# biscuitzb/COEB-SLAM

Measured on AMD Instinct MI355X. Metric: frames/sec ORB extract+match @640x480/1000 kp; 1/2/4/8 GPU + %HBM roofline, higher is better.
Workload: dtype u8; 1 GPU; 640x480, 8-level pyramid, 1000 kp, extract + Hamming match to prev frame (BASELINE configs[1]); width=640, height=480, nfeatures=1000, nlevels=8, halo_frames_per_rank=1, pipelines_per_gpu=3, streams_per_gpu=1, ranks=single, parallelism=frame-sharded x1 (no collectives), hw_queues=4, side_stream=own, side_stream_created=with the context

## Files before the change

coeb-slam_amd/csrc/coeb_extract.hip:

```cpp
#include <type_traits>
#include <cmath>
#include <hip/hip_runtime.h>

#include "coeb_internal.hpp"

namespace {

constexpr int kThreads = 256;
constexpr int kWaves = kThreads / 64;

__device__ __forceinline__ int lane_id() { return __lane_id(); }
__device__ __forceinline__ int wave_id() { return __builtin_amdgcn_readfirstlane(threadIdx.x >> 6); }
__device__ __forceinline__ void wave_sync_lds()
{
    __builtin_amdgcn_fence(__ATOMIC_RELEASE, "wavefront");
    __builtin_amdgcn_wave_barrier();
    __builtin_amdgcn_fence(__ATOMIC_ACQUIRE, "wavefront");
}
typedef unsigned int u32x4 __attribute__((ext_vector_type(4)));

__device__ __forceinline__ uint64_t lanemask_lt() { return (1ull << lane_id()) - 1ull; }

__device__ __forceinline__ int wave_sum(int v)
{
// ... 345 lines not shown
    uint32_t sel[2], coef[2];
    const int d0 = min((int)cx, dw - 1);
    const uint32_t wb = (uint32_t)(xofs[d0] & ~3);
    const uint32_t wb1 = (uint32_t)min((int)wb + 4, sp - 4);
#pragma unroll
    for (int k = 0; k < 2; k++) {
        const int d = min((int)cx + k, dw - 1);
        const int o = xofs[d] - (int)wb;
        const int a = alpha[d];
        const uint32_t a0 = d >= xmax ? 2048u : (uint32_t)(a & 0xFFFF), a1 = d >= xmax ? 0u : (uint32_t)a >> 16;
        coef[k] = a0 | (a1 << 16);
        sel[k] = (uint32_t)o | 0x0c00u | ((uint32_t)(o + 1) << 16) | 0x0c000000u;
    }
    const __amdgpu_buffer_rsrc_t rs =
        __builtin_amdgcn_make_buffer_rsrc((void*)(src + (int64_t)f * src_fs), 0, 0x7fffffff, 0x00020000);
    const __amdgpu_buffer_rsrc_t rd =
        __builtin_amdgcn_make_buffer_rsrc((void*)(dst + (int64_t)f * dst_fs), 0, 0x7fffffff, 0x00020000);
    const bool edge = ox + PR_COLS > dw - 1, tail = ox + PR_COLS > xs;
    const int* band = bands + (oy / PR_ROWS) * kPyrBandInts;
    const int4 bd = *reinterpret_cast<const int4*>(band);
    if (bd.x != kPyrBandGeneric) {
#define COEB_PYR_PATTERN(P, LAST) pyr_rows_pattern<P, LAST>(rs, rd, wb, wb1, sel, coef, band, bd.y, bd.z, sp, dp, cx, dw, xs)
        if (edge || tail) {
            switch (bd.x) {
            case 0: COEB_PYR_PATTERN(0, true); break;
            case 1: COEB_PYR_PATTERN(1, true); break;
            case 2: COEB_PYR_PATTERN(2, true); break;
            case 3: COEB_PYR_PATTERN(3, true); break;
            default: COEB_PYR_PATTERN(4, true); break;
            }
        } else {
            switch (bd.x) {
            case 0: COEB_PYR_PATTERN(0, false); break;
            case 1: COEB_PYR_PATTERN(1, false); break;
            case 2: COEB_PYR_PATTERN(2, false); break;
            case 3: COEB_PYR_PATTERN(3, false); break;
            default: COEB_PYR_PATTERN(4, false); break;
            }
        }
#undef COEB_PYR_PATTERN
        return;
    }
    uint32_t w[PR_ROWS][4];
#pragma unroll
    for (int r = 0; r < PR_ROWS; r++) {
        const int4 yr = yrow[min(oy + r, dh - 1)];
        w[r][0] = __builtin_amdgcn_raw_buffer_load_b32(rs, wb, yr.x, 0);
        w[r][1] = __builtin_amdgcn_raw_buffer_load_b32(rs, wb1, yr.x, 0);
        w[r][2] = __builtin_amdgcn_raw_buffer_load_b32(rs, wb, yr.y, 0);
        w[r][3] = __builtin_amdgcn_raw_buffer_load_b32(rs, wb1, yr.y, 0);
    }
    if (tail) {
        if (edge) pyr_rows_out<true, true>(w, sel, coef, yrow, rd, oy, dh, cx, dw, xs);
        else pyr_rows_out<true, false>(w, sel, coef, yrow, rd, oy, dh, cx, dw, xs);
    } else {
        if (edge) pyr_rows_out<false, true>(w, sel, coef, yrow, rd, oy, dh, cx, dw, xs);
        else pyr_rows_out<false, false>(w, sel, coef, yrow, rd, oy, dh, cx, dw, xs);
    }
}

constexpr int kBlurCols = 56;

__device__ __forceinline__ int reflect101(int p, int len)
{
    if (len == 1) return 0;
    while (p < 0 || p >= len) p = p < 0 ? -p : 2 * len - p - 2;
    return p;
}

struct BlurWork {
    int L;
    int item0, item1;
    int item_off[COEB_MAXL + 1];
    int nstrips[COEB_MAXL];
    int bh[COEB_MAXL];
    int nquads[COEB_MAXL];
    int brows;
};


template <bool kRemap = true>
__device__ __forceinline__ int2 block_xy()
{
    const int gx = gridDim.x;
    if (!kRemap) return make_int2(blockIdx.x, blockIdx.y);
    const int n = gx * gridDim.y, p = blockIdx.x + gx * blockIdx.y;
    const int q = n >> 3, r = n & 7, x = p & 7, k = p >> 3;
    const int lg = x * q + min(x, r) + k;
    return make_int2(lg % gx, lg / gx);
}

__device__ __forceinline__ uint32_t dpp_shr1(uint32_t v)
{
    return (uint32_t)__builtin_amdgcn_mov_dpp((int)v, 0x111, 0xf, 0xf, false);
}
__device__ __forceinline__ uint32_t dpp_shl1(uint32_t v)
{
    return (uint32_t)__builtin_amdgcn_mov_dpp((int)v, 0x101, 0xf, 0xf, false);
}

__device__ __forceinline__ int reflect_row(int r, int h)
{
    int rr = r < 0 ? -r : r;
    rr = rr >= h ? 2 * h - 2 - rr : rr;
    return rr < 0 ? 0 : rr;
}

constexpr int kBlurQuad = 4 * kBlurCols;
constexpr int kBlurPitch = kBlurQuad + 16;
static_assert(kBlurQuad % 16 == 0, "a wave item must cover whole 16-column tiles");

__global__ __launch_bounds__(kThreads) void k_blur_rows(const Plan* __restrict__ P, ExtractBufs b, BlurWork bw)
{
    __shared__ __attribute__((aligned(16))) uint8_t s_tile[kWaves][8 * kBlurPitch];
    const int2 bxy = block_xy();
    const int f = bxy.y;
    const int item = bw.item0 + bxy.x * kWaves + wave_id();
    if (item >= bw.item1) return;
    int l = 0;
    while (l + 1 < bw.L && item >= bw.item_off[l + 1]) l++;
    const int it = item - bw.item_off[l];
    const int nq = bw.nquads[l];
    const int quad = it % nq, band = it / nq;
    const LevelGeom& g = P->lv[l];
    const int w = g.w, h = g.h, sp = g.pitch, dp = g.bpitch;
    const int lane = lane_id(), grp = lane >> 4, gl = lane & 15;
    const int y0 = band * bw.brows, y1 = min(h, y0 + bw.brows);
    const int x = (quad * 4 + grp) * kBlurCols - 4 + gl * 4;
    const bool produce = gl >= 1 && gl <= 14 && x < w;
    const int xbase = quad * kBlurQuad;
    uint8_t* tl = s_tile[wave_id()];
    int cq[4];
#pragma unroll
    for (int q = 0; q < 4; q++) cq[q] = reflect101(min(x + q, w + 2), w);
    const int a = min(min(min(cq[0], cq[1]), min(cq[2], cq[3])), w - 4);
    const uint32_t sel0 = 0x0c000c00u | (uint32_t)(cq[0] - a) | ((uint32_t)(cq[1] - a) << 16);
    const uint32_t sel1 = 0x0c000c00u | (uint32_t)(cq[2] - a) | ((uint32_t)(cq[3] - a) << 16);
    const __amdgpu_buffer_rsrc_t rs =
        __builtin_amdgcn_make_buffer_rsrc((void*)level_ptr(P, b, f, l), 0, 0x7fffffff, 0x00020000);
    const __amdgpu_buffer_rsrc_t rd =
        __builtin_amdgcn_make_buffer_rsrc((void*)(b.blur + (int64_t)f * P->blur_stride + g.blur_off), 0, 0x7fffffff,
                                          0x00020000);
    const int k0 = P->gauss[0], k1 = P->gauss[1], k2 = P->gauss[2], k3 = P->gauss[3];
    const us2 K0 = pk2(k0, k0), K1 = pk2(k1, k1), K2 = pk2(k2, k2), K3 = pk2(k3, k3);
    const us2 W_l01_0 = pk2(0, k0), W_l23_0 = pk2(k1, k2), W_c01_0 = pk2(k3, k2), W_c23_0 = pk2(k1, k0);
    const us2 W_l23_1 = pk2(k0, k1), W_c01_1 = pk2(k2, k3), W_c23_1 = pk2(k2, k1), W_r01_1 = pk2(k0, 0);
    const us2 W_l23_2 = pk2(0, k0), W_c01_2 = pk2(k1, k2), W_c23_2 = pk2(k3, k2), W_r01_2 = pk2(k1, k0);
    const us2 W_c01_3 = pk2(k0, k1), W_c23_3 = pk2(k2, k3), W_r01_3 = pk2(k2, k1), W_r23_3 = pk2(k0, 0);
    const uint32_t rnd = 1u << 15;
    const int nfull = (y1 - y0) >> 3, tail = (y1 - y0) & 7;
    uint32_t R0[8], R1[8];
    auto take = [&](int s, uint32_t raw) {
        R0[s] = __builtin_amdgcn_perm(0u, raw, sel0);
        R1[s] = __builtin_amdgcn_perm(0u, raw, sel1);
    };
    typedef __attribute__((address_space(3))) uint32_t* lds_u32;
    lds_u32 trow = (lds_u32)(tl + (produce ? x - xbase : kBlurQuad + 8 * (grp & 1) + 4 * (gl & 1)));
    asm volatile("" : "+v"(trow));
    auto out_row = [&](int s, int k) {
        const int s0 = (s + 2) & 7, s1 = (s + 3) & 7, s2 = (s + 4) & 7, s3 = (s + 5) & 7, s4 = (s + 6) & 7,
                  s5 = (s + 7) & 7, s6 = s;
        const us2 v01 = K3 * as_us2(R0[s3]) + K2 * (as_us2(R0[s2]) + as_us2(R0[s4])) +
                        K1 * (as_us2(R0[s1]) + as_us2(R0[s5])) + K0 * (as_us2(R0[s0]) + as_us2(R0[s6]));
        const us2 v23 = K3 * as_us2(R1[s3]) + K2 * (as_us2(R1[s2]) + as_us2(R1[s4])) +
                        K1 * (as_us2(R1[s1]) + as_us2(R1[s5])) + K0 * (as_us2(R1[s0]) + as_us2(R1[s6]));
        const uint32_t V01 = as_u32(v01), V23 = as_u32(v23);
        const us2 L01 = as_us2(dpp_shr1(V01)), L23 = as_us2(dpp_shr1(V23));
        const us2 R01 = as_us2(dpp_shl1(V01)), R23 = as_us2(dpp_shl1(V23));
        uint32_t a0 = __builtin_amdgcn_udot2(L01, W_l01_0, rnd, false);
        a0 = __builtin_amdgcn_udot2(L23, W_l23_0, a0, false);
        a0 = __builtin_amdgcn_udot2(v01, W_c01_0, a0, false);
        a0 = __builtin_amdgcn_udot2(v23, W_c23_0, a0, false);
        uint32_t a1 = __builtin_amdgcn_udot2(L23, W_l23_1, rnd, false);
        a1 = __builtin_amdgcn_udot2(v01, W_c01_1, a1, false);
        a1 = __builtin_amdgcn_udot2(v23, W_c23_1, a1, false);
        a1 = __builtin_amdgcn_udot2(R01, W_r01_1, a1, false);
        uint32_t a2 = __builtin_amdgcn_udot2(L23, W_l23_2, rnd, false);
        a2 = __builtin_amdgcn_udot2(v01, W_c01_2, a2, false);
        a2 = __builtin_amdgcn_udot2(v23, W_c23_2, a2, false);
        a2 = __builtin_amdgcn_udot2(R01, W_r01_2, a2, false);
        uint32_t a3 = __builtin_amdgcn_udot2(v01, W_c01_3, rnd, false);
        a3 = __builtin_amdgcn_udot2(v23, W_c23_3, a3, false);
        a3 = __builtin_amdgcn_udot2(R01, W_r01_3, a3, false);
        a3 = __builtin_amdgcn_udot2(R23, W_r23_3, a3, false);
        const uint32_t p01 = __builtin_amdgcn_perm(a1, a0, 0x0c0c0602u);
        const uint32_t p23 = __builtin_amdgcn_perm(a3, a2, 0x06020c0cu);
        trow[k * (kBlurPitch / 4)] = p01 | p23;
    };
    const int c1 = lane + 64;
    const bool st0 = xbase + 16 * (lane >> 3) < dp;
    const bool st1 = c1 < kBlurQuad / 2 && xbase + 16 * (c1 >> 3) < dp;
    const uint8_t* const tsrc0 = tl + (lane & 7) * kBlurPitch + 16 * (lane >> 3);
    const uint8_t* const tsrc1 = tl + (c1 & 7) * kBlurPitch + 16 * (c1 >> 3);
    const int tdst = (xbase >> 4) * 128 + 16 * lane;
    int so_d = __builtin_amdgcn_readfirstlane((int)blur_tile_off(0, y0, dp));
    const int so_dstep = __builtin_amdgcn_readfirstlane((dp >> 4) * 128);
    auto flush = [&]() {
        wave_sync_lds();
        if (st0) __builtin_amdgcn_raw_buffer_store_b128(*reinterpret_cast<const u32x4*>(tsrc0), rd, tdst, so_d, 0);
        if (st1)
            __builtin_amdgcn_raw_buffer_store_b128(*reinterpret_cast<const u32x4*>(tsrc1), rd, tdst + 16 * 64, so_d, 0);
        wave_sync_lds();
        so_d += so_dstep;
    };
    auto band_rows = [&](auto reflect) {
        constexpr bool kReflect = decltype(reflect)::value;
        int r = y0 - 3;
        int so = __builtin_amdgcn_readfirstlane((y0 - 3) * sp);
        auto load_row = [&]() -> uint32_t {
            int o;
            if constexpr (kReflect) {
                o = __builtin_amdgcn_readfirstlane(reflect_row(r, h) * sp);
                r++;
            } else {
                o = so;
                so += sp;
            }
            return __builtin_amdgcn_raw_buffer_load_b32(rs, a, o, 0);
        };
        uint32_t pro[6], nxt[8];
#pragma unroll
        for (int s = 0; s < 6; s++) pro[s] = load_row();
#pragma unroll
        for (int k = 0; k < 8; k++) nxt[k] = 0u;
        if (nfull > 0) {
#pragma unroll
            for (int k = 0; k < 8; k++) nxt[k] = load_row();
        } else {
#pragma unroll
            for (int k = 0; k < 7; k++)
                if (k < tail) nxt[k] = load_row();
        }
#pragma unroll
        for (int s = 0; s < 6; s++) take(s, pro[s]);
        for (int blk = 0; blk < nfull; blk++) {
            uint32_t raw[8];
#pragma unroll
            for (int k = 0; k < 8; k++) raw[k] = nxt[k];
            if (blk + 1 < nfull) {
#pragma unroll
                for (int k = 0; k < 8; k++) nxt[k] = load_row();
            } else {
#pragma unroll
                for (int k = 0; k < 7; k++)
                    if (k < tail) nxt[k] = load_row();
            }
#pragma unroll
            for (int k = 0; k < 8; k++) {
                take((6 + k) & 7, raw[k]);
                out_row((6 + k) & 7, k);
            }
            flush();
        }
        if (tail) {
#pragma unroll
            for (int k = 0; k < 7; k++) {
                if (k >= tail) break;
                take((6 + k) & 7, nxt[k]);
                out_row((6 + k) & 7, k);
            }
            flush();
        }
    };
    if (y0 >= 3 && y1 + 2 < h) band_rows(std::false_type());
    else band_rows(std::true_type());
}

typedef const __attribute__((address_space(3))) uint8_t* lds_cu8;
typedef const __attribute__((address_space(3))) uint32_t* lds_cu32;

__device__ __forceinline__ void ring16(const uint8_t* c, int st, int p[16])
{
    p[0] = c[3 * st];      p[1] = c[3 * st + 1];  p[2] = c[2 * st + 2];  p[3] = c[st + 3];
    p[4] = c[3];           p[5] = c[-st + 3];     p[6] = c[-2 * st + 2]; p[7] = c[-3 * st + 1];
    p[8] = c[-3 * st];     p[9] = c[-3 * st - 1]; p[10] = c[-2 * st - 2]; p[11] = c[-st - 3];
    p[12] = c[-3];         p[13] = c[st - 3];     p[14] = c[2 * st - 2]; p[15] = c[3 * st - 1];
}

__device__ __forceinline__ int corner_strength(const uint8_t* c, int st)
{
    int p[16];
    ring16(c, st, p);
    const int v = c[0];
    int d[16];
#pragma unroll
    for (int k = 0; k < 16; k++) d[k] = v - p[k];
    int t[16];
#pragma unroll
    for (int k = 0; k < 16; k++) t[k] = min(min(d[k], d[(k + 1) & 15]), d[(k + 2) & 15]);
    int A = -1000;
#pragma unroll
    for (int k = 0; k < 16; k++) A = max(A, min(min(t[k], t[(k + 3) & 15]), t[(k + 6) & 15]));
#pragma unroll
    for (int k = 0; k < 16; k++) t[k] = max(max(d[k], d[(k + 1) & 15]), d[(k + 2) & 15]);
    int Bm = 1000;
#pragma unroll
    for (int k = 0; k < 16; k++) Bm = min(Bm, max(max(t[k], t[(k + 3) & 15]), t[(k + 6) & 15]));
    return max(A, -Bm);
}

constexpr int kFastRowBytes = 72;
constexpr int kFastRowBytesM = 96;
constexpr int kFastGuard = 16;
constexpr int kFastEnt = 128;
constexpr int kFastSurv = 4 * 64 + 8;
constexpr int kFastCorners = 256;
constexpr int kFastLists = kFastSurv;
static_assert(kFastRowBytesM * 64 <= 4 * 4096 && kFastRowBytes * 64 <= 4 * 4096, "k_fast entry offset field");


__device__ __forceinline__ bool fast_pretest(const uint8_t* c, int st, int t)
{
    const int v = c[0];
    const int lo = v - t, hi = v + t;
    auto cls = [&](int x) { return (x < lo ? 1 : 0) | (x > hi ? 2 : 0); };
    int d = cls(c[3 * st]) | cls(c[-3 * st]);
    d &= cls(c[2 * st + 2]) | cls(c[-2 * st - 2]);
    d &= cls(c[3]) | cls(c[-3]);
    d &= cls(c[-2 * st + 2]) | cls(c[2 * st - 2]);
    return d != 0;
}

__device__ __forceinline__ uint32_t win_lo(uint32_t a, uint32_t b, int s)
{
    return __builtin_amdgcn_perm(b, a, 0x0c000c00u | (uint32_t)s | ((uint32_t)(s + 1) << 16));
}
__device__ __forceinline__ uint32_t win_hi(uint32_t a, uint32_t b, int s)
{
    return __builtin_amdgcn_perm(b, a, 0x0c000c00u | (uint32_t)(s + 2) | ((uint32_t)(s + 3) << 16));
}

__device__ __forceinline__ us2 pk_min(us2 a, us2 b) { return __builtin_elementwise_min(a, b); }
__device__ __forceinline__ us2 pk_max(us2 a, us2 b) { return __builtin_elementwise_max(a, b); }
__device__ __forceinline__ us2 pk_subs(us2 a, us2 b) { return __builtin_elementwise_sub_sat(a, b); }

__device__ __forceinline__ us2 pk_max3(us2 a, us2 b, us2 c)
{
    uint32_t r;
    asm("v_pk_maximum3_f16 %0, %1, %2, %3" : "=v"(r) : "v"(as_u32(a)), "v"(as_u32(b)), "v"(as_u32(c)));
    return as_us2(r);
}
__device__ __forceinline__ us2 pk_min3(us2 a, us2 b, us2 c)
{
    uint32_t r;
    asm("v_pk_minimum3_f16 %0, %1, %2, %3" : "=v"(r) : "v"(as_u32(a)), "v"(as_u32(b)), "v"(as_u32(c)));
    return as_us2(r);
}

__device__ __forceinline__ uint32_t pretest_half(us2 v, us2 p0, us2 p8, us2 p2, us2 p10, us2 p4, us2 p12, us2 p6,
                                                 us2 p14, us2 T)
{
    const us2 md = pk_max3(pk_min(p0, p8), pk_min(p2, p10), pk_max(pk_min(p4, p12), pk_min(p6, p14)));
    const us2 mb = pk_min3(pk_max(p0, p8), pk_max(p2, p10), pk_min(pk_max(p4, p12), pk_max(p6, p14)));
    return as_u32(pk_subs(pk_max(pk_subs(v, md), pk_subs(mb, v)), T));
}

template <bool kMax, bool S1, bool S2>
__device__ __forceinline__ uint32_t pk3(uint32_t a, uint32_t b, uint32_t c)
{
    uint32_t r;
#define COEB_PK3(OP, SEL) asm(OP " %0, %1, %2, %3" SEL : "=v"(r) : "v"(a), "v"(b), "v"(c))
    if constexpr (kMax) {
        if constexpr (!S1 && !S2) COEB_PK3("v_pk_maximum3_f16", "");
        else if constexpr (!S1 && S2) COEB_PK3("v_pk_maximum3_f16", " op_sel:[0,0,1] op_sel_hi:[1,1,0]");
        else if constexpr (S1 && !S2) COEB_PK3("v_pk_maximum3_f16", " op_sel:[0,1,0] op_sel_hi:[1,0,1]");
        else COEB_PK3("v_pk_maximum3_f16", " op_sel:[0,1,1] op_sel_hi:[1,0,0]");
    } else {
        if constexpr (!S1 && !S2) COEB_PK3("v_pk_minimum3_f16", "");
        else if constexpr (!S1 && S2) COEB_PK3("v_pk_minimum3_f16", " op_sel:[0,0,1] op_sel_hi:[1,1,0]");
        else if constexpr (S1 && !S2) COEB_PK3("v_pk_minimum3_f16", " op_sel:[0,1,0] op_sel_hi:[1,0,1]");
        else COEB_PK3("v_pk_minimum3_f16", " op_sel:[0,1,1] op_sel_hi:[1,0,0]");
    }
#undef COEB_PK3
    return r;
}

__device__ __forceinline__ uint32_t arc_max_min_pk(const uint32_t Q[8])
{
    uint32_t M3[8], M9[8];
#pragma unroll
    for (int k = 0; k < 6; k++) M3[k] = pk3<false, false, false>(Q[k], Q[k + 1], Q[k + 2]);
    M3[6] = pk3<false, false, true>(Q[6], Q[7], Q[0]);
    M3[7] = pk3<false, true, true>(Q[7], Q[0], Q[1]);
    M9[0] = pk3<false, false, false>(M3[0], M3[3], M3[6]);
    M9[1] = pk3<false, false, false>(M3[1], M3[4], M3[7]);
#pragma unroll
    for (int k = 2; k < 5; k++) M9[k] = pk3<false, false, true>(M3[k], M3[k + 3], M3[k - 2]);
#pragma unroll
    for (int k = 5; k < 8; k++) M9[k] = pk3<false, true, true>(M3[k], M3[k - 5], M3[k - 2]);
    const uint32_t A = pk3<true, false, false>(M9[0], M9[1], M9[2]);
    const uint32_t B = pk3<true, false, false>(M9[3], M9[4], M9[5]);
    return pk3<true, false, false>(M9[6], M9[7], pk3<true, false, false>(A, B, A));
}

template <int st>
__device__ __forceinline__ int corner_strength_pos2(const uint8_t* c, int t)
{
    lds_cu8 b = (lds_cu8)c - (3 * st + 1);
    asm volatile("" : "+v"(b));
    constexpr int o = 3 * st + 1;
    constexpr int off[16] = {o + 3 * st, o + 3 * st + 1, o + 2 * st + 2, o + st + 3, o + 3, o - st + 3, o - 2 * st + 2,
                             o - 3 * st + 1, 1, 0, o - 2 * st - 2, o - st - 3, o - 3, o + st - 3, o + 2 * st - 2,
                             o + 3 * st - 1};
    us2 Qv[8];
#pragma unroll
    for (int k = 0; k < 8; k++) { Qv[k].x = b[off[k]]; Qv[k].y = b[off[k + 8]]; }
    const int v = b[o];
    uint32_t Q[8];
#pragma unroll
    for (int k = 0; k < 8; k++) Q[k] = as_u32(Qv[k]);
    auto lo = [](uint32_t x) { return (int)(x & 0xFFFFu); };
    auto hi = [](uint32_t x) { return (int)(x >> 16); };
    const int md = max(max(min(lo(Q[0]), hi(Q[0])), min(lo(Q[2]), hi(Q[2]))),
                       max(min(lo(Q[4]), hi(Q[4])), min(lo(Q[6]), hi(Q[6]))));
    const int mb = min(min(max(lo(Q[0]), hi(Q[0])), max(lo(Q[2]), hi(Q[2]))),
                       min(max(lo(Q[4]), hi(Q[4])), max(lo(Q[6]), hi(Q[6]))));
    const bool dark = md < v - t, bright = mb > v + t;
    const uint32_t mask = dark ? 0x00FF00FFu : 0u;
    uint32_t Qx[8];
#pragma unroll
    for (int k = 0; k < 8; k++) Qx[k] = Q[k] ^ mask;
    const uint32_t X = arc_max_min_pk(Qx);
    int M = max(lo(X), hi(X)) - (v ^ (int)(mask & 0xFFu));
    if (__builtin_expect(__ballot(dark && bright) != 0, 0)) {
        if (dark && bright) {
            const uint32_t Y = arc_max_min_pk(Q);
            M = max(M, max(lo(Y), hi(Y)) - v);
        }
    }
    return M;
}

template <int RB>
__device__ __forceinline__ void fast_pretest4_raw(const uint8_t* c, int t, uint32_t& lo, uint32_t& hi)
{
    constexpr int st = RB;
    lds_cu32 w = (lds_cu32)(c - 3 * st);
    asm volatile("" : "+v"(w));
    constexpr int o = 3 * st / 4;
    const uint32_t a0 = w[o - 1], b0 = w[o], c0 = w[o + 1];
    const uint32_t ap = w[o + 2 * st / 4 - 1], bp = w[o + 2 * st / 4], cp = w[o + 2 * st / 4 + 1];
    const uint32_t am = w[o - 2 * st / 4 - 1], bm = w[o - 2 * st / 4], cm = w[o - 2 * st / 4 + 1];
    const uint32_t u3 = w[o + 3 * st / 4];
    const uint32_t d3 = w[0];
    const us2 T = pk2(t, t);
    lo = pretest_half(
        as_us2(__builtin_amdgcn_perm(0u, b0, 0x0c010c00u)), as_us2(__builtin_amdgcn_perm(0u, u3, 0x0c010c00u)),
        as_us2(__builtin_amdgcn_perm(0u, d3, 0x0c010c00u)), as_us2(win_lo(bp, cp, 2)), as_us2(win_lo(am, bm, 2)),
        as_us2(win_lo(b0, c0, 3)), as_us2(win_lo(a0, b0, 1)), as_us2(win_lo(bm, cm, 2)), as_us2(win_lo(ap, bp, 2)), T);
    hi = pretest_half(
        as_us2(__builtin_amdgcn_perm(0u, b0, 0x0c030c02u)), as_us2(__builtin_amdgcn_perm(0u, u3, 0x0c030c02u)),
        as_us2(__builtin_amdgcn_perm(0u, d3, 0x0c030c02u)), as_us2(win_hi(bp, cp, 2)), as_us2(win_hi(am, bm, 2)),
        as_us2(win_hi(b0, c0, 3)), as_us2(win_hi(a0, b0, 1)), as_us2(win_hi(bm, cm, 2)), as_us2(win_hi(ap, bp, 2)), T);
}

template <int RB>
__device__ __forceinline__ int fast_mi(int o, int mp)
{
    if constexpr (RB == kFastRowBytesM) {
        return o + 45;
    } else {
        const int yy = (int)((unsigned)o / (unsigned)RB);
        return (yy - 2) * mp + (o - yy * RB) - 3;
    }
}

__device__ __forceinline__ int nms_keep(const uint8_t* Ms, int mi, int mp, int t, int* sc_out)
{
    const int M = Ms[mi];
    if (M <= t) return 0;
    const int sc = M - 1;
    bool kept = true;
#pragma unroll
    for (int dy = -1; dy <= 1; dy++)
#pragma unroll
        for (int dx = -1; dx <= 1; dx++) {
            if (dx == 0 && dy == 0) continue;
            const int Mn = Ms[mi + dy * mp + dx];
            const int ns = Mn > t ? Mn - 1 : 0;
            kept = kept && (sc > ns);
        }
    *sc_out = sc;
    return kept ? 1 : 0;
}

__device__ __forceinline__ int mbcnt(uint64_t m)
{
    return (int)__builtin_amdgcn_mbcnt_hi((uint32_t)(m >> 32), __builtin_amdgcn_mbcnt_lo((uint32_t)m, 0u));
}
__device__ __forceinline__ int uniform(int v) { return __builtin_amdgcn_readfirstlane(v); }

constexpr int kFastPass = 12;

struct FastCellGeom {
    const uint8_t* img;
    int pitch, x0, y0, rw, rh, nwords;
    bool vec;
    bool words;
};

struct FastRegs {
    u32x4 v0, v1, v2;
};

__device__ __forceinline__ FastCellGeom fast_geom(const Plan* P, const ExtractBufs& b, int f, const CellDesc& c)
{
    FastCellGeom G;
    const LevelGeom& g = P->lv[c.level];
    G.img = level_ptr(P, b, f, c.level);
    G.pitch = g.pitch;
    G.x0 = c.x0; G.y0 = c.y0; G.rw = c.rw; G.rh = c.rh;
    G.nwords = (1 + c.rw + 3) >> 2;
    G.vec = ((g.pitch | (int)reinterpret_cast<uintptr_t>(G.img)) & 15) == 0 && G.nwords <= 12 && c.rh <= 48;
    G.words = (g.pitch & 3) == 0 && G.nwords <= 15 && c.rh <= 4 * kFastPass;
    return G;
}

__device__ __forceinline__ void fast_prefetch(const FastCellGeom& G, FastRegs& R)
{
    const int lane = lane_id();
    if (G.vec) {
        const uint8_t* base = G.img + (int64_t)G.y0 * G.pitch + ((G.x0 - 1) & ~15) + 16 * (lane & 3);
        const int r = lane >> 2;
        R.v0 = *reinterpret_cast<const u32x4*>(base + (int64_t)min(r, G.rh - 1) * G.pitch);
        R.v1 = *reinterpret_cast<const u32x4*>(base + (int64_t)min(r + 16, G.rh - 1) * G.pitch);
        R.v2 = *reinterpret_cast<const u32x4*>(base + (int64_t)min(r + 32, G.rh - 1) * G.pitch);
    }
}

__device__ __attribute__((aligned(64))) const uint8_t g_fast_zero[64] = {0};

__device__ __forceinline__ void fast_dma(const FastCellGeom& G, uint8_t* roi)
{
    typedef __attribute__((address_space(3))) void* lds_vp;
    const int lane = lane_id();
    const int nq = 6 * G.rh;
    const uint8_t* row0 = G.img + (int64_t)G.y0 * G.pitch + (G.x0 - 1);
#pragma unroll
    for (int i = 0; i < 5; i++) {
        if (64 * i < nq) {
            const int q = 64 * i + lane;
            const int r = (q * 171) >> 10;
            const int k = q - 6 * r;
            const uint8_t* src = k < 3 ? row0 + r * G.pitch + 16 * k : g_fast_zero;
            if (q < nq) __builtin_amdgcn_global_load_lds((const void*)src, (lds_vp)(roi + 1024 * i), 16, 0, 0);
        }
    }
}
__device__ __forceinline__ void fast_dma_wait() { asm volatile("s_waitcnt vmcnt(0)" ::: "memory"); }

template <int RB>
__device__ __forceinline__ void fast_stage(const FastCellGeom& G, const FastRegs& R, uint8_t* roi)
{
    const int lane = lane_id();
    if (G.vec) {
        const int sh = (G.x0 - 1) & 15;
        const int r = lane >> 2, c = lane & 3;
        uint8_t* d = roi + r * RB + 16 * c - sh;
        if (r < G.rh) __builtin_memcpy(d, &R.v0, 16);
        if (r + 16 < G.rh) __builtin_memcpy(d + 16 * RB, &R.v1, 16);
        if (r + 32 < G.rh) __builtin_memcpy(d + 32 * RB, &R.v2, 16);
        if constexpr (RB == kFastRowBytesM) {
            asm volatile("" ::: "memory");
            uint8_t* z = roi + r * RB + 48 + 16 * c;
            const uint4 zero = make_uint4(0, 0, 0, 0);
            if (c < 3 && r < G.rh) *reinterpret_cast<uint4*>(z) = zero;
            if (c < 3 && r + 16 < G.rh) *reinterpret_cast<uint4*>(z + 16 * RB) = zero;
            if (c < 3 && r + 32 < G.rh) *reinterpret_cast<uint4*>(z + 32 * RB) = zero;
        }
    } else if (G.words) {
        const int gx = G.x0 - 1;
        const int kw = min(lane & 15, G.nwords);
        const uint32_t* wbase = reinterpret_cast<const uint32_t*>(G.img + (int64_t)G.y0 * G.pitch + (gx & ~3)) + kw;
        const int pw = G.pitch >> 2;
        const int npass = (G.rh + 3) >> 2;
        uint32_t q0[kFastPass];
#pragma unroll
        for (int i = 0; i < kFastPass; i++)
            if (i < npass) q0[i] = wbase[min((lane >> 4) + 4 * i, G.rh - 1) * pw];
        const int al = (G.x0 - 1) & 3;
#pragma unroll
        for (int i = 0; i < kFastPass; i++) {
            if (i < npass) {
                const uint32_t q1 = dpp_shl1(q0[i]);
                const int yy = (lane >> 4) + 4 * i;
                if (yy < G.rh && (lane & 15) < G.nwords)
                    *reinterpret_cast<uint32_t*>(roi + yy * RB + 4 * (lane & 15)) =
                        __builtin_amdgcn_alignbyte(q1, q0[i], (uint32_t)al);
            }
        }
    } else if ((G.pitch & 3) == 0) {
        const int gx = G.x0 - 1;
        const int al = gx & 3;
        const uint8_t* base = G.img + (int64_t)G.y0 * G.pitch + (gx & ~3);
        for (int yy = lane >> 4; yy < G.rh; yy += 4)
            for (int k = lane & 15; k < G.nwords; k += 16) {
                const uint32_t* q = reinterpret_cast<const uint32_t*>(base + (int64_t)yy * G.pitch) + k;
                *reinterpret_cast<uint32_t*>(roi + yy * RB + 4 * k) =
                    __builtin_amdgcn_alignbyte(q[1], q[0], (uint32_t)al);
            }
    } else {
        for (int yy = lane >> 4; yy < G.rh; yy += 4)
            for (int xx = lane & 15; xx < G.rw; xx += 16)
                roi[yy * RB + 1 + xx] = G.img[(int64_t)(G.y0 + yy) * G.pitch + G.x0 + xx];
    }
}

__host__ __device__ inline int fast_rb(const Plan& P) { return P.max_roi_w <= 46 ? kFastRowBytesM : kFastRowBytes; }
__host__ __device__ inline int fast_slab(const Plan& P, int rb) { return (rb * P.max_roi_h + 15) & ~15; }
__host__ __device__ inline int fast_mp(const Plan& P) { return (P.max_roi_w - 6 + 2 + 3) & ~3; }
__host__ __device__ inline int fast_ms_slab(const Plan& P, int rb)
{
    return rb == kFastRowBytesM ? 0 : (fast_mp(P) * (P.max_roi_h - 4) + 15) & ~15;
}
__host__ __device__ inline int fast_wave_lds(const Plan& P, int rb)
{
    return kFastGuard + fast_slab(P, rb) + fast_ms_slab(P, rb) + 2 * (kFastLists + kFastCorners + kFastEnt);
}

#define FC_MARK(v) long long v = COEB_FAST_CLOCK ? (long long)clock64() : 0
__device__ unsigned long long g_fast_clk[256 * 8];
#define FC_SLOT(slot) g_fast_clk[(blockIdx.x & 255) * 8 + (slot)]
#define FC_ADD(slot, t0) do { if (COEB_FAST_CLOCK && lane_id() == 0) atomicAdd(&FC_SLOT(slot), (unsigned long long)((long long)clock64() - (t0))); } while (0)

template <int RB>
__device__ __forceinline__ void fast_cell(const Plan* P, const ExtractBufs& b, int f, int cidx, const CellDesc& c,
                                          int th_ini, int th_min, const uint8_t* roi, uint8_t* Ms, uint16_t* surv,
                                          uint16_t* corn, uint16_t* ent)
{
    constexpr int sh = 1;
    const int lane = lane_id();
    const LevelGeom& g = P->lv[c.level];
    const int rw = c.rw, rh = c.rh;
    const int ww = rw - 6, wh = rh - 6;
    const int mp = RB == kFastRowBytesM ? RB : fast_mp(*P);
    const int npix = ww > 0 && wh > 0 ? ww * wh : 0;
    int ne = 0, nc = 0;
    const int ngrp = (ww + 3) >> 2;
    const int lpr_log = ngrp > 8 ? 4 : 3;
    const int cg = lane & ((1 << lpr_log) - 1), rsub = lane >> lpr_log;
    const int rpi = 64 >> lpr_log;
    const uint32_t vmask4 = (1u << min(max(ww - 4 * cg, 0), 4)) - 1u;
    int o = (rsub + 3) * RB + 4 + 4 * cg;
    const uint32_t one2 = 0x00010001u;
    FC_MARK(t_scan);
    long long t_str = 0;
    auto flush = [&]() {
        FC_MARK(t_s0);
        wave_sync_lds();
        for (int e0 = 0; e0 < ne; e0 += 64) {
            const int e = e0 + lane;
            const uint32_t en = e < ne ? (uint32_t)ent[e] : 0u;
            const uint32_t m = en >> 12;
            const int cnt = __popc(m);
            const uint64_t b0 = __ballot(cnt & 1), b1 = __ballot(cnt & 2), b2 = __ballot(cnt & 4);
            int q = mbcnt(b0) + 2 * mbcnt(b1) + 4 * mbcnt(b2);
            const int ns = uniform((int)__popcll(b0) + 2 * (int)__popcll(b1) + 4 * (int)__popcll(b2));
            const int ob = (int)(en & 0xFFFu) << 2;
#pragma unroll
            for (int k = 0; k < 4; k++)
                if ((m >> k) & 1u) surv[q++] = (uint16_t)(ob + k);
            surv[ns] = surv[ns > 0 ? ns - 1 : 0];
            wave_sync_lds();
            for (int s0 = 0; s0 < ns; s0 += 64) {
                const int si = s0 + lane;
                int oo = 0, M = 0;
                if (si < ns) {
                    oo = surv[si];
                    M = corner_strength_pos2<RB>(&roi[oo], th_min);
                }
                const bool isc = si < ns && M > th_min;
                if (isc) Ms[fast_mi<RB>(oo, mp)] = (uint8_t)M;
                const uint64_t mc = __ballot(isc);
                if (isc) {
                    const int qq = nc + mbcnt(mc);
                    if (qq < kFastCorners) corn[qq] = (uint16_t)oo;
                }
                nc = uniform(nc + (int)__popcll(mc));
            }
            wave_sync_lds();
        }
        ne = 0;
        if (COEB_FAST_CLOCK) t_str += (long long)clock64() - t_s0;
    };
    for (int r0 = 0; npix > 0 && r0 < wh; r0 += rpi, o += rpi * RB) {
        uint32_t lo, hi;
        fast_pretest4_raw<RB>(&roi[o], th_min, lo, hi);
        uint32_t s01, s23;
        asm("v_pk_min_u16 %0, %1, %2" : "=v"(s01) : "v"(lo), "v"(one2));
        asm("v_pk_min_u16 %0, %1, %2" : "=v"(s23) : "v"(hi), "v"(one2));
        const uint32_t t2 = s01 | (s23 << 2);
        const uint32_t m4 = (t2 | (t2 >> 15)) & (rsub < wh - r0 ? vmask4 : 0u);
        const uint64_t mk = __ballot(m4 != 0u);
        if (mk) {
            if (m4) ent[ne + mbcnt(mk)] = (uint16_t)(((uint32_t)o >> 2) | (m4 << 12));
            ne = uniform(ne + (int)__popcll(mk));
        }
        if (ne > kFastEnt - 64 || r0 + rpi >= wh) flush();
    }
    FC_ADD(1, t_scan + t_str);
    if (COEB_FAST_CLOCK && lane_id() == 0) atomicAdd(&FC_SLOT(2), (unsigned long long)t_str);
    FC_MARK(t_nms);
    uint32_t* out = b.cand + ((int64_t)f * P->ncells + cidx) * P->cell_cap;
    int nkept = 0;
    for (int pass = 0; pass < 2; pass++) {
        const int t = pass == 0 ? th_ini : th_min;
        int running = 0;
        if (nc <= kFastCorners) {
            for (int e0 = 0; e0 < nc; e0 += 64) {
                const int e = e0 + lane;
                int oo = 0, sc = 0, kept = 0;
                if (e < nc) {
                    oo = corn[e];
                    kept = nms_keep(Ms, fast_mi<RB>(oo, mp), mp, t, &sc);
                }
                const uint64_t m = __ballot(kept);
                if (kept) {
                    const int q = running + mbcnt(m);
                    const int yy = oo / RB, xx = oo - yy * RB - sh;
                    if (q < P->cell_cap) out[q] = pack_key(xx + c.j * g.wcell, yy + c.i * g.hcell, sc);
                    else atomicOr(b.err, 2);
                }
                running = uniform(running + __popcll(m));
            }
        } else {
            int row0 = 0, col0 = 0;
            for (int base = 0; base < npix; base += 64) {
                int col = col0 + lane, row = row0;
                while (col >= ww) { col -= ww; row++; }
                int sc = 0, kept = 0;
                const int mi = RB == kFastRowBytesM ? (row + 3) * RB + col + 4 + 45 : (row + 1) * mp + col + 1;
                if (base + lane < npix) kept = nms_keep(Ms, mi, mp, t, &sc);
                const uint64_t m = __ballot(kept);
                if (kept) {
                    const int q = running + mbcnt(m);
                    if (q < P->cell_cap) out[q] = pack_key(col + 3 + c.j * g.wcell, row + 3 + c.i * g.hcell, sc);
                    else atomicOr(b.err, 2);
                }
                running = uniform(running + __popcll(m));
                col0 += 64;
                while (col0 >= ww) { col0 -= ww; row0++; }
            }
        }
        nkept = running;
        if (nkept > 0) break;
    }
    if (lane == 0) b.cand_n[(int64_t)f * P->ncells + cidx] = min(nkept, P->cell_cap);
    FC_ADD(3, t_nms);
    if (COEB_FAST_CLOCK && lane == 0) { atomicAdd(&FC_SLOT(5), 1ull); atomicAdd(&FC_SLOT(6), (unsigned long long)nc); }
}

__device__ __forceinline__ CellDesc load_cell(const CellDesc* __restrict__ cells, int i)
{
    const int4 r = reinterpret_cast<const int4*>(cells)[i];
    CellDesc c;
    c.level = (int16_t)(r.x & 0xFFFF); c.pad = 0;
    c.x0 = (int16_t)(r.y & 0xFFFF); c.y0 = (int16_t)(r.y >> 16);
    c.rw = (int16_t)(r.z & 0xFFFF); c.rh = (int16_t)(r.z >> 16);
    c.i = (int16_t)(r.w & 0xFFFF); c.j = (int16_t)(r.w >> 16);
    return c;
}

template <int RB>
#ifndef COEB_FAST_MINWG
#define COEB_FAST_MINWG 6
#endif
__global__ __launch_bounds__(kThreads, COEB_FAST_MINWG) void k_fast(const Plan* __restrict__ P, ExtractBufs b,
                                                       const CellDesc* __restrict__ cells,
                                                       int cell0, int cell1)
{
    extern __shared__ __attribute__((aligned(16))) uint8_t smem[];
    const int wv = wave_id(), lane = lane_id();
    const int slab = fast_slab(*P, RB), ms_slab = fast_ms_slab(*P, RB);
    uint8_t* wbase = smem + (size_t)wv * fast_wave_lds(*P, RB) + kFastGuard;
    uint8_t* roi = wbase;
    uint8_t* Ms = RB == kFastRowBytesM ? wbase : wbase + slab;
    uint16_t* surv = reinterpret_cast<uint16_t*>(wbase + slab + ms_slab);
    uint16_t* corn = surv + kFastLists;
    uint16_t* ent = corn + kFastCorners;
    const int2 bxy = block_xy<false>();
    const int f = bxy.y;
    const int cidx = cell0 + bxy.x * kWaves + wv;
    if (cidx >= cell1) return;
    const int area = b.dyn[f].area_flag;
    const int th_ini = area ? 30 : 20, th_min = area ? 10 : 7;
    const CellDesc c = load_cell(cells, cidx);
    const FastCellGeom G = fast_geom(P, b, f, c);
    const bool dma = RB == kFastRowBytesM && c.rh <= 48;
    FastRegs R;
    if (dma) fast_dma(G, roi);
    else fast_prefetch(G, R);
    FC_MARK(t_all);
    FC_MARK(t_st);
    if (dma) fast_dma_wait();
    else fast_stage<RB>(G, R, roi);
    if (RB == kFastRowBytesM) {
        if (!G.vec && !dma)
        for (int i = lane; i < 3 * (c.rh - 4); i += 64) {
            const int row = 2 + i / 3;
            reinterpret_cast<uint4*>(Ms + row * RB + 48)[i - 3 * (row - 2)] = make_uint4(0, 0, 0, 0);
        }
    } else {
        for (int i = lane; i < ms_slab / 16; i += 64) reinterpret_cast<uint4*>(Ms)[i] = make_uint4(0, 0, 0, 0);
    }
    wave_sync_lds();
    FC_ADD(0, t_st);
    fast_cell<RB>(P, b, f, cidx, c, th_ini, th_min, roi, Ms, surv, corn, ent);
    FC_ADD(4, t_all);
}

__device__ __forceinline__ void lds_barrier()
{
    __builtin_amdgcn_fence(__ATOMIC_RELEASE, "workgroup", "local");
    __builtin_amdgcn_s_barrier();
    __builtin_amdgcn_fence(__ATOMIC_ACQUIRE, "workgroup", "local");
}

struct NodeRef {
    int* start; int* cnt; int* alloc; int* buf; int4* rect;
};

struct OctLds {
    int* work; int4* cnt; int* base; int* rank; int* push; uint8_t* dead;
    NodeRef set[2];
    uint32_t* keys[2];
    size_t set_stride;
};

__device__ __forceinline__ OctLds oct_lds(uint8_t* smem, int W, int KL)
{
    OctLds o;
    size_t off = 0;
    o.cnt = reinterpret_cast<int4*>(smem + off); off += (size_t)W * 16;
    o.work = reinterpret_cast<int*>(smem + off); off += (size_t)W * 4;
    o.base = reinterpret_cast<int*>(smem + off); off += (size_t)W * 4;
    o.rank = reinterpret_cast<int*>(smem + off); off += (size_t)W * 4;
    o.push = reinterpret_cast<int*>(smem + off); off += (size_t)W * 4;
    for (int s = 0; s < 2; s++) {
        o.set[s].rect = reinterpret_cast<int4*>(smem + off); off += (size_t)W * 16;
        o.set[s].start = reinterpret_cast<int*>(smem + off); off += (size_t)W * 4;
        o.set[s].cnt = reinterpret_cast<int*>(smem + off); off += (size_t)W * 4;
        o.set[s].alloc = reinterpret_cast<int*>(smem + off); off += (size_t)W * 4;
        o.set[s].buf = reinterpret_cast<int*>(smem + off); off += (size_t)W * 4;
    }
    o.set_stride = (size_t)W * 32;
    o.keys[0] = reinterpret_cast<uint32_t*>(smem + off); off += (size_t)KL * 4;
    o.keys[1] = reinterpret_cast<uint32_t*>(smem + off); off += (size_t)KL * 4;
    o.dead = smem + off;
    return o;
}

__device__ __forceinline__ NodeRef nref(const OctLds& O, int s)
{
    NodeRef r = O.set[0];
    const size_t d = s ? O.set_stride : 0;
    r.rect = reinterpret_cast<int4*>(reinterpret_cast<uint8_t*>(r.rect) + d);
    r.start = reinterpret_cast<int*>(reinterpret_cast<uint8_t*>(r.start) + d);
    r.cnt = reinterpret_cast<int*>(reinterpret_cast<uint8_t*>(r.cnt) + d);
    r.alloc = reinterpret_cast<int*>(reinterpret_cast<uint8_t*>(r.alloc) + d);
    r.buf = reinterpret_cast<int*>(reinterpret_cast<uint8_t*>(r.buf) + d);
    return r;
}

__device__ __forceinline__ int quadrant(uint32_t k, int sx, int sy)
{
    const int x = key_x(k), y = key_y(k);
    return x < sx ? (y < sy ? 0 : 2) : (y < sy ? 1 : 3);
}

__device__ __forceinline__ int4 wave_count_quadrants(const uint32_t* src, int s, int n, int sx, int sy)
{
    int c0 = 0, c1 = 0, c2 = 0, c3 = 0;
    const int lane = lane_id();
    for (int base = 0; base < n; base += 64) {
        const int i = base + lane;
        const bool v = i < n;
        const int q = v ? quadrant(src[s + i], sx, sy) : -1;
        c0 += __popcll(__ballot(q == 0));
        c1 += __popcll(__ballot(q == 1));
        c2 += __popcll(__ballot(q == 2));
        c3 += __popcll(__ballot(q == 3));
    }
    return make_int4(c0, c1, c2, c3);
}

__device__ __forceinline__ void wave_scatter_quadrants_at(const uint32_t* src, uint32_t* dst, int s, int n,
                                                          int sx, int sy, int4 r)
{
    int r0 = r.x, r1 = r.y, r2 = r.z, r3 = r.w;
    const int lane = lane_id();
    const uint64_t lt = lanemask_lt();
    for (int base = 0; base < n; base += 64) {
        const int i = base + lane;
        const bool v = i < n;
        const uint32_t k = v ? src[s + i] : 0u;
        const int q = v ? quadrant(k, sx, sy) : -1;
        const uint64_t m0 = __ballot(q == 0), m1 = __ballot(q == 1), m2 = __ballot(q == 2), m3 = __ballot(q == 3);
        if (v) {
            const uint64_t mq = q == 0 ? m0 : q == 1 ? m1 : q == 2 ? m2 : m3;
            const int rq = q == 0 ? r0 : q == 1 ? r1 : q == 2 ? r2 : r3;
            dst[rq + __popcll(mq & lt)] = k;
        }
        r0 += __popcll(m0); r1 += __popcll(m1); r2 += __popcll(m2); r3 += __popcll(m3);
    }
}

__device__ __forceinline__ void wave_scatter_quadrants(const uint32_t* src, uint32_t* dst, int s, int n,
                                                       int sx, int sy, int4 c)
{
    wave_scatter_quadrants_at(src, dst, s, n, sx, sy,
                              make_int4(s, s + c.x, s + c.x + c.y, s + c.x + c.y + c.z));
}

__device__ __forceinline__ int4 lane_count_quadrants(const uint32_t* src, int s, int n, int sx, int sy)
{
    int c0 = 0, c1 = 0, c2 = 0, c3 = 0;
    for (int i = 0; i < n; i++) {
        const int q = quadrant(src[s + i], sx, sy);
        c0 += q == 0; c1 += q == 1; c2 += q == 2; c3 += q == 3;
    }
    return make_int4(c0, c1, c2, c3);
}

__device__ __forceinline__ void lane_scatter_quadrants(const uint32_t* src, uint32_t* dst, int s, int n, int sx,
                                                       int sy, int4 c)
{
    int r0 = s, r1 = s + c.x, r2 = s + c.x + c.y, r3 = s + c.x + c.y + c.z;
    for (int i = 0; i < n; i++) {
        const uint32_t k = src[s + i];
        const int q = quadrant(k, sx, sy);
        const int r = q == 0 ? r0++ : q == 1 ? r1++ : q == 2 ? r2++ : r3++;
        dst[r] = k;
    }
}

template <int G>
__device__ __forceinline__ int4 team_count_quadrants(const uint32_t* src, int s, int n, int sx, int sy)
{
    int c0 = 0, c1 = 0, c2 = 0, c3 = 0;
    for (int i = lane_id() & (G - 1); i < n; i += G) {
        const int q = quadrant(src[s + i], sx, sy);
        c0 += q == 0; c1 += q == 1; c2 += q == 2; c3 += q == 3;
    }
#pragma unroll
    for (int o = 1; o < G; o <<= 1) {
        c0 += __shfl_xor(c0, o, 64); c1 += __shfl_xor(c1, o, 64);
        c2 += __shfl_xor(c2, o, 64); c3 += __shfl_xor(c3, o, 64);
    }
    return make_int4(c0, c1, c2, c3);
}

template <int G>
__device__ __forceinline__ void team_scatter_quadrants(const uint32_t* src, uint32_t* dst, int s, int n, int sx,
                                                       int sy, int4 c)
{
    int r0 = s, r1 = s + c.x, r2 = s + c.x + c.y, r3 = s + c.x + c.y + c.z;
    const int lane = lane_id(), gl = lane & (G - 1);
    const uint64_t tm = ((1ull << G) - 1ull) << (lane & ~(G - 1));
    for (int base = 0; base < n; base += G) {
        const int i = base + gl;
        const bool v = i < n;
        const uint32_t k = v ? src[s + i] : 0u;
        const int q = v ? quadrant(k, sx, sy) : -1;
        const uint64_t m0 = __ballot(q == 0) & tm, m1 = __ballot(q == 1) & tm;
        const uint64_t m2 = __ballot(q == 2) & tm, m3 = __ballot(q == 3) & tm;
        if (v) {
            const uint64_t mq = q == 0 ? m0 : q == 1 ? m1 : q == 2 ? m2 : m3;
            const int rq = q == 0 ? r0 : q == 1 ? r1 : q == 2 ? r2 : r3;
            dst[rq + mbcnt(mq)] = k;
        }
        r0 += __popcll(m0); r1 += __popcll(m1); r2 += __popcll(m2); r3 += __popcll(m3);
    }
}

template <int NT>
__device__ __forceinline__ int oct_team(int nd, int avg)
{
    int best = 64, bc = 0x7fffffff;
#pragma unroll
    for (int gi = 0; gi < 4; gi++) {
        const int G = 64 >> (2 * gi);
        const int c = ((nd * G + NT - 1) / NT) * ((avg + G - 1) / G);
        if (c < bc) { bc = c; best = G; }
    }
    return best;
}

__device__ __forceinline__ void child_rect(const int4 p, int q, int4* out, int* sx, int* sy)
{
    const int hx = (int)ceilf((float)(p.z - p.x) / 2);
    const int hy = (int)ceilf((float)(p.w - p.y) / 2);
    const int mx = p.x + hx, my = p.y + hy;
    *sx = mx; *sy = my;
    if (q == 0) *out = make_int4(p.x, p.y, mx, my);
    else if (q == 1) *out = make_int4(mx, p.y, p.z, my);
// ... 940 lines not shown
```

Measured before the change: 394,100 frames/s.

## Weaken FAST pretest to four compass pixels, enlarge entry buffer, hoist LDS pointer

The vectorized FAST pretest now checks only the four compass pixels (0,4,8,12) instead of all eight even-indexed circle pixels, so it loads fewer LDS words and issues fewer packed min/max ops per 4-pixel group. The entry buffer grows from 128 to 192 so flushes happen less often. The LDS window pointer is hoisted and advanced incrementally, and the last-row validity mask is precomputed. The weaker pretest lets more candidates through to the full corner-strength stage, trading scan work for more survivor processing, and the larger entry buffer costs extra LDS.

```diff
diff --git a/coeb-slam_amd/csrc/coeb_extract.hip b/coeb-slam_amd/csrc/coeb_extract.hip
--- a/coeb-slam_amd/csrc/coeb_extract.hip
+++ b/coeb-slam_amd/csrc/coeb_extract.hip
@@ -671,7 +671,7 @@
 constexpr int kFastRowBytes = 72;
 constexpr int kFastRowBytesM = 96;
 constexpr int kFastGuard = 16;
-constexpr int kFastEnt = 128;
+constexpr int kFastEnt = 192;
 constexpr int kFastSurv = 4 * 64 + 8;
 constexpr int kFastCorners = 256;
 constexpr int kFastLists = kFastSurv;
@@ -703,24 +703,10 @@
 __device__ __forceinline__ us2 pk_max(us2 a, us2 b) { return __builtin_elementwise_max(a, b); }
 __device__ __forceinline__ us2 pk_subs(us2 a, us2 b) { return __builtin_elementwise_sub_sat(a, b); }
 
-__device__ __forceinline__ us2 pk_max3(us2 a, us2 b, us2 c)
-{
-    uint32_t r;
-    asm("v_pk_maximum3_f16 %0, %1, %2, %3" : "=v"(r) : "v"(as_u32(a)), "v"(as_u32(b)), "v"(as_u32(c)));
-    return as_us2(r);
-}
-__device__ __forceinline__ us2 pk_min3(us2 a, us2 b, us2 c)
-{
-    uint32_t r;
-    asm("v_pk_minimum3_f16 %0, %1, %2, %3" : "=v"(r) : "v"(as_u32(a)), "v"(as_u32(b)), "v"(as_u32(c)));
-    return as_us2(r);
-}
-
-__device__ __forceinline__ uint32_t pretest_half(us2 v, us2 p0, us2 p8, us2 p2, us2 p10, us2 p4, us2 p12, us2 p6,
-                                                 us2 p14, us2 T)
-{
-    const us2 md = pk_max3(pk_min(p0, p8), pk_min(p2, p10), pk_max(pk_min(p4, p12), pk_min(p6, p14)));
-    const us2 mb = pk_min3(pk_max(p0, p8), pk_max(p2, p10), pk_min(pk_max(p4, p12), pk_max(p6, p14)));
+__device__ __forceinline__ uint32_t pretest_half(us2 v, us2 p0, us2 p8, us2 p4, us2 p12, us2 T)
+{
+    const us2 md = pk_max(pk_min(p0, p8), pk_min(p4, p12));
+    const us2 mb = pk_min(pk_max(p0, p8), pk_max(p4, p12));
     return as_u32(pk_subs(pk_max(pk_subs(v, md), pk_subs(mb, v)), T));
 }
 
@@ -801,26 +787,19 @@
 }
 
 template <int RB>
-__device__ __forceinline__ void fast_pretest4_raw(const uint8_t* c, int t, uint32_t& lo, uint32_t& hi)
-{
-    constexpr int st = RB;
-    lds_cu32 w = (lds_cu32)(c - 3 * st);
-    asm volatile("" : "+v"(w));
-    constexpr int o = 3 * st / 4;
+__device__ __forceinline__ void fast_pretest4_raw(lds_cu32 w, int t, uint32_t& lo, uint32_t& hi)
+{
+    constexpr int o = 3 * RB / 4;
     const uint32_t a0 = w[o - 1], b0 = w[o], c0 = w[o + 1];
-    const uint32_t ap = w[o + 2 * st / 4 - 1], bp = w[o + 2 * st / 4], cp = w[o + 2 * st / 4 + 1];
-    const uint32_t am = w[o - 2 * st / 4 - 1], bm = w[o - 2 * st / 4], cm = w[o - 2 * st / 4 + 1];
-    const uint32_t u3 = w[o + 3 * st / 4];
+    const uint32_t u3 = w[2 * o];
     const uint32_t d3 = w[0];
     const us2 T = pk2(t, t);
     lo = pretest_half(
         as_us2(__builtin_amdgcn_perm(0u, b0, 0x0c010c00u)), as_us2(__builtin_amdgcn_perm(0u, u3, 0x0c010c00u)),
-        as_us2(__builtin_amdgcn_perm(0u, d3, 0x0c010c00u)), as_us2(win_lo(bp, cp, 2)), as_us2(win_lo(am, bm, 2)),
-        as_us2(win_lo(b0, c0, 3)), as_us2(win_lo(a0, b0, 1)), as_us2(win_lo(bm, cm, 2)), as_us2(win_lo(ap, bp, 2)), T);
+        as_us2(__builtin_amdgcn_perm(0u, d3, 0x0c010c00u)), as_us2(win_lo(b0, c0, 3)), as_us2(win_lo(a0, b0, 1)), T);
     hi = pretest_half(
         as_us2(__builtin_amdgcn_perm(0u, b0, 0x0c030c02u)), as_us2(__builtin_amdgcn_perm(0u, u3, 0x0c030c02u)),
-        as_us2(__builtin_amdgcn_perm(0u, d3, 0x0c030c02u)), as_us2(win_hi(bp, cp, 2)), as_us2(win_hi(am, bm, 2)),
-        as_us2(win_hi(b0, c0, 3)), as_us2(win_hi(a0, b0, 1)), as_us2(win_hi(bm, cm, 2)), as_us2(win_hi(ap, bp, 2)), T);
+        as_us2(__builtin_amdgcn_perm(0u, d3, 0x0c030c02u)), as_us2(win_hi(b0, c0, 3)), as_us2(win_hi(a0, b0, 1)), T);
 }
 
 template <int RB>
@@ -1011,6 +990,9 @@
     const int rpi = 64 >> lpr_log;
     const uint32_t vmask4 = (1u << min(max(ww - 4 * cg, 0), 4)) - 1u;
     int o = (rsub + 3) * RB + 4 + 4 * cg;
+    lds_cu32 pw = (lds_cu32)(roi + o - 3 * RB);
+    const int r0_last = wh > 0 ? (wh - 1) & -rpi : 0;
+    const uint32_t vmask4_last = rsub < wh - r0_last ? vmask4 : 0u;
     const uint32_t one2 = 0x00010001u;
     FC_MARK(t_scan);
     long long t_str = 0;
@@ -1052,14 +1034,14 @@
         ne = 0;
         if (COEB_FAST_CLOCK) t_str += (long long)clock64() - t_s0;
     };
-    for (int r0 = 0; npix > 0 && r0 < wh; r0 += rpi, o += rpi * RB) {
+    for (int r0 = 0; npix > 0 && r0 < wh; r0 += rpi, o += rpi * RB, pw += rpi * RB / 4) {
         uint32_t lo, hi;
-        fast_pretest4_raw<RB>(&roi[o], th_min, lo, hi);
+        fast_pretest4_raw<RB>(pw, th_min, lo, hi);
         uint32_t s01, s23;
         asm("v_pk_min_u16 %0, %1, %2" : "=v"(s01) : "v"(lo), "v"(one2));
         asm("v_pk_min_u16 %0, %1, %2" : "=v"(s23) : "v"(hi), "v"(one2));
         const uint32_t t2 = s01 | (s23 << 2);
-        const uint32_t m4 = (t2 | (t2 >> 15)) & (rsub < wh - r0 ? vmask4 : 0u);
+        const uint32_t m4 = (t2 | (t2 >> 15)) & (r0 == r0_last ? vmask4_last : vmask4);
         const uint64_t mk = __ballot(m4 != 0u);
         if (mk) {
             if (m4) ent[ne + mbcnt(mk)] = (uint16_t)(((uint32_t)o >> 2) | (m4 << 12));
```

New measurement: 399,700 frames/s (median of 6 runs). 1.4% higher.
